# theoad/ot-vae-lightning

Hardware: AMD Instinct MI355X
Metric: training images/sec (whole node) + OT-loss rel-err vs CPU ref (higher is better)
Workload: dtype f32; 1 GPU; MNIST-32 CNN VAE (capacity 8, latent 128x1x1, residual=add) + GaussianPrior(loss_coeff=0.1): fwd+bwd+Adam + latent Gaussian statistics update, hipGraph replay; per_gpu_batch=1024, global_batch=1024, parallelism=single GPU

## Files before the change

### ot_vae_lightning_amd/csrc/conv.hip

```cpp
#include "common.h"
#include "conv_small.h"
#include "conv_tile.h"
#include "conv_wtile.h"

static inline Geom to_geom(const otvae_conv_geom* g) {
    Geom r = {g->N, g->Hs, g->Ws, g->Cs, g->up, g->Ho, g->Wo, g->Cn, g->KH, g->KW, g->stride, g->pad};
    return r;
}

static int check_geom(const otvae_conv_geom* g, const char* who) {
    OTVAE_REQUIRE(g != nullptr, "%s: geom is NULL", who);
    OTVAE_REQUIRE(g->N > 0 && g->Hs > 0 && g->Ws > 0 && g->Cs > 0 && g->Cn > 0, "%s: non-positive dims", who);
    OTVAE_REQUIRE(g->up == 1 || g->up == 2, "%s: up must be 1 or 2 (got %d)", who, g->up);
    OTVAE_REQUIRE(g->stride == 1 || g->stride == 2, "%s: stride must be 1 or 2 (got %d)", who, g->stride);
    OTVAE_REQUIRE(!(g->up == 2 && g->stride != 1), "%s: up-sampling with stride != 1 unsupported", who);
    OTVAE_REQUIRE(g->KH >= 1 && g->KH <= 7 && g->KW >= 1 && g->KW <= 7, "%s: kernel size out of range", who);
    int Hu = g->Hs * g->up, Wu = g->Ws * g->up;
    int ho = (Hu + 2 * g->pad - g->KH) / g->stride + 1, wo = (Wu + 2 * g->pad - g->KW) / g->stride + 1;
    OTVAE_REQUIRE(ho == g->Ho && wo == g->Wo, "%s: output size mismatch: geom says %dx%d, conv gives %dx%d", who,
                  g->Ho, g->Wo, ho, wo);
    OTVAE_REQUIRE((int64_t)g->N * Hu * Wu * imax(g->Cs, g->Cn) < (int64_t)1 << 31, "%s: tensor too large for 32-bit indexing",
                  who);
    OTVAE_REQUIRE(g->Cs <= 2048 && g->Cn <= 2048, "%s: more than 2048 channels unsupported", who);
    if (g->stride == 2) OTVAE_REQUIRE(g->Hs % 2 == 0 && g->Ws % 2 == 0, "%s: stride 2 needs even input size", who);
// ... 42 lines not shown
        n = rdiv(t, g.Hs, rd.iHs, rd.small);
        const int sy = t - (unsigned)n * g.Hs;
        iy = 2 * sy + (child >> 1);
        ix = 2 * sx + (child & 1);
    } else if (g.stride == 2) {
        const int W2 = g.Ws >> 1, H2 = g.Hs >> 1;
        const unsigned t = rdiv(row, W2, rd.iW2, rd.small);
        const int jx = row - t * W2;
        n = rdiv(t, H2, rd.iH2, rd.small);
        const int jy = t - (unsigned)n * H2;
        iy = 2 * jy + py;
        ix = 2 * jx + px;
    } else {
        const unsigned t = rdiv(row, g.Ws, rd.iWs, rd.small);
        ix = row - t * g.Ws;
        n = rdiv(t, g.Hs, rd.iHs, rd.small);
        iy = t - (unsigned)n * g.Hs;
    }
}

template <int NT>
struct GemmSmem {
    static constexpr int BN = 16 * NT;
    static constexpr int LDA = KC + 2;
    static constexpr int LDB = BN + ((BN % 32 == 0) ? 16 : 0);
    static constexpr size_t as_off = 0;
    static constexpr size_t bs_off = as_off + sizeof(float) * 2 * TM * LDA;
    static constexpr size_t red_off = bs_off + sizeof(float) * 2 * KC * LDB;
    static constexpr size_t tap_off = red_off + sizeof(double) * 4 * 2 * BN;
    static constexpr size_t row_off = tap_off + sizeof(int) * (3 * MAX_TAPS + 1);
    static constexpr size_t bytes = (row_off + sizeof(int) * 3 * TM + 15) / 16 * 16;
};

template <int MODE, int NT, bool VEC, bool UT = false>
__device__ __forceinline__ void conv_gemm_body(char* __restrict__ smem, const Geom& g, const float* __restrict__ S,
                                               const float* __restrict__ scale, const float* __restrict__ shift, int relu,
                                               const float* __restrict__ Bmat,
                                               const float* __restrict__ bias, const float* __restrict__ res,
                                               float* __restrict__ y,
                                               const float* __restrict__ xin, const float* __restrict__ mean,
                                               const float* __restrict__ invstd, float* __restrict__ gv,
                                               double* __restrict__ partial, int CsPad, int bx, int by, int bz, int gx,
                                               int gz) {
    using SM = GemmSmem<NT>;
    constexpr int BN = SM::BN;
    constexpr int LDA = SM::LDA;
    constexpr int LDB = SM::LDB;
    constexpr int NB_ELEMS = KC * BN / 256;
    float(*As)[TM * LDA] = reinterpret_cast<float(*)[TM * LDA]>(smem + SM::as_off);
    float(*Bs)[KC * LDB] = reinterpret_cast<float(*)[KC * LDB]>(smem + SM::bs_off);
    double* red = reinterpret_cast<double*>(smem + SM::red_off);
    int* tap_dy = reinterpret_cast<int*>(smem + SM::tap_off);
    int* tap_dx = tap_dy + MAX_TAPS;
    int* tap_w = tap_dx + MAX_TAPS;
    int& s_ntaps = tap_w[MAX_TAPS];
    int* row_n = reinterpret_cast<int*>(smem + SM::row_off);
    int* row_y = row_n + TM;
    int* row_x = row_y + TM;

    const int tid = threadIdx.x, lane = tid & 63, wave = tid >> 6;
    const int r16 = lane & 15, kq = lane >> 4;
    const int cls = bz, py = cls >> 1, px = cls & 1;
    const int Hu = g.Hs * g.up, Wu = g.Ws * g.up;
    const int CK = MODE == 0 ? g.Cs : g.Cn;
    const int NC = MODE == 0 ? g.Cn : g.Cs;
    const int n0 = by * BN;
    const int lim_y = MODE == 0 ? Hu : g.Ho * g.stride, lim_x = MODE == 0 ? Wu : g.Wo * g.stride;
    const int sh = MODE == 0 ? g.up - 1 : g.stride - 1;
    const int srcH = MODE == 0 ? g.Hs : g.Ho, srcW = MODE == 0 ? g.Ws : g.Wo;
    const unsigned rows = MODE == 0 ? (unsigned)g.N * g.Ho * g.Wo
                                    : (g.stride == 2 ? (unsigned)g.N * (g.Hs >> 1) * (g.Ws >> 1) : (unsigned)g.N * Hu * Wu);
    const unsigned ntiles = (rows + TM - 1) / TM;
    const RowDiv rd = make_rowdiv(g, rows);

    if (tid == 0) {
        int nt = 0;
        for (int kh = 0; kh < g.KH; ++kh)
            for (int kw = 0; kw < g.KW; ++kw) {
                bool ok;
                int dy, dx;
                if (MODE == 0) {
                    dy = kh - g.pad;
                    dx = kw - g.pad;
                    ok = (dy + (g.Ho - 1) * g.stride >= 0) && (dy < Hu) && (dx + (g.Wo - 1) * g.stride >= 0) && (dx < Wu);
                } else {
                    dy = g.pad - kh;
                    dx = g.pad - kw;
                    ok = true;
                    if (g.stride == 2) ok = (((py + dy) & 1) == 0) && (((px + dx) & 1) == 0);
                    ok = ok && (Hu - 1 + dy >= 0) && (dy < lim_y) && (Wu - 1 + dx >= 0) && (dx < lim_x);
                }
                if (ok) {
                    tap_dy[nt] = dy;
                    tap_dx[nt] = dx;
                    tap_w[nt] = kh * g.KW + kw;
                    ++nt;
                }
            }
        s_ntaps = nt;
    }
    __syncthreads();
    const int ntaps = s_ntaps;
    const int K = ntaps * CK;
    const int nch = (K + KC - 1) / KC;
    const float inv_ck = 1.0f / (float)CK;
    const int cpt = CK / KC;
    const float inv_cpt = 1.0f / (float)(cpt > 0 ? cpt : 1);

    const int a_kl = tid & 31, a_r0 = tid >> 5;

    double s1[NT], s2[NT];
#pragma unroll
    for (int j = 0; j < NT; ++j) s1[j] = s2[j] = 0.0;

    for (unsigned tile = bx; tile < ntiles; tile += gx) {
        __syncthreads();
        if (tid < TM) {
            const unsigned row = tile * TM + tid;
            int n = -1, ry = 0, rx = 0;
            if (row < rows) {
                if (MODE == 0) {
                    const unsigned t = rdiv(row, g.Wo, rd.iWo, rd.small);
                    const int ox = row - t * g.Wo;
                    n = rdiv(t, g.Ho, rd.iHo, rd.small);
                    const int oy = t - (unsigned)n * g.Ho;
                    ry = oy * g.stride;
                    rx = ox * g.stride;
                } else {
                    int iy, ix;
                    dgrad_row_to_pos(g, rd, row, py, px, n, iy, ix);
                    ry = iy;
                    rx = ix;
                }
            }
            row_n[tid] = n;
            row_y[tid] = ry;
            row_x[tid] = rx;
        }
        __syncthreads();

        f32x4 acc[NT];
#pragma unroll
        for (int j = 0; j < NT; ++j) acc[j] = (f32x4){0.f, 0.f, 0.f, 0.f};

        constexpr int NBV = (8 * BN + 255) / 256;
        float areg[8], breg[NB_ELEMS];
        float4 areg4[2], breg4[NBV];
        float4 a_sc4 = make_float4(1.f, 1.f, 1.f, 1.f), a_sh4 = make_float4(0.f, 0.f, 0.f, 0.f);
        int a_ok = 0;
        float a_sc = 1.f, a_sh = 0.f;
        const int v_k4 = tid & 7, v_r0 = tid >> 3;
        int vr_n[2], vr_y[2], vr_x[2];
        if constexpr (VEC) {
// ... 247 lines not shown
                const int buf = ch & 1;
                if (ch + 1 < nch) stage_load(ch + 1);
                {
                    const float* Ab = &As[buf][(wave * 16 + r16) * LDA + kq];
                    const float* Bb = &Bs[buf][kq * LDB + r16];
                    float av[KC / 4], bv[KC / 4][NT];
#pragma unroll
                    for (int ks = 0; ks < KC / 4; ++ks) {
                        av[ks] = Ab[ks * 4];
#pragma unroll
                        for (int j = 0; j < NT; ++j) bv[ks][j] = Bb[ks * 4 * LDB + j * 16];
                    }
#pragma unroll
                    for (int ks = 0; ks < KC / 4; ++ks)
#pragma unroll
                        for (int j = 0; j < NT; ++j) acc[j] = mfma16(av[ks], bv[ks][j], acc[j]);
                }
                if (ch + 1 < nch) stage_store(buf ^ 1);
                __syncthreads();
            }
        }

        const unsigned row0 = tile * TM + wave * 16 + kq * 4;
        if (MODE == 0) {
#pragma unroll
            for (int j = 0; j < NT; ++j) {
                const int col = n0 + j * 16 + r16;
                if (col < g.Cn) {
                    const float bv = bias ? bias[col] : 0.f;
#pragma unroll
                    for (int r = 0; r < 4; ++r) {
                        const unsigned pm = row0 + r;
                        if (pm < rows) {
                            const size_t o = (size_t)pm * g.Cn + col;
                            float v = acc[j][r] + bv;
                            if (res) v += res[o];
                            y[o] = v;
                            if (partial) {
                                s1[j] += (double)v;
                                s2[j] += (double)v * (double)v;
                            }
                        }
                    }
                }
            }
        } else {
#pragma unroll
            for (int j = 0; j < NT; ++j) {
                const int col = n0 + j * 16 + r16;
                if (col >= g.Cs) continue;
                const float sc = scale ? scale[col] : 1.f, shf = scale ? shift[col] : 0.f;
                const float mu = mean ? mean[col] : 0.f, is = mean ? invstd[col] : 0.f;
                if (g.up == 2) {
                    if (row0 < rows) {
                        const unsigned parent = row0 >> 2;
                        float val = (acc[j][0] + acc[j][1]) + (acc[j][2] + acc[j][3]);
                        const size_t o = (size_t)parent * g.Cs + col;
                        float xv = 0.f;
                        if (relu || mean) xv = xin[o];
                        if (relu) {
                            const float v = scale ? fmaf(xv, sc, shf) : xv;
                            val = v > 0.f ? val : 0.f;
                        }
                        gv[o] = val;
                        if (mean) {
                            s1[j] += (double)val;
                            s2[j] += (double)val * (double)((xv - mu) * is);
                        }
                    }
                } else {
#pragma unroll
                    for (int r = 0; r < 4; ++r) {
                        const unsigned rr = row0 + r;
                        if (rr < rows) {
                            size_t o;
                            if (g.stride == 1) {
                                o = (size_t)rr * g.Cs + col;
                            } else {
                                int pn, piy, pix;
                                dgrad_row_to_pos(g, rd, rr, py, px, pn, piy, pix);
                                o = ((size_t)((unsigned)pn * g.Hs + piy) * g.Ws + pix) * g.Cs + col;
                            }
                            float val = acc[j][r];
                            float xv = 0.f;
                            if (relu || mean) xv = xin[o];
                            if (relu) {
                                const float v = scale ? fmaf(xv, sc, shf) : xv;
                                val = v > 0.f ? val : 0.f;
                            }
                            gv[o] = val;
                            if (mean) {
                                s1[j] += (double)val;
                                s2[j] += (double)val * (double)((xv - mu) * is);
                            }
                        }
                    }
                }
            }
        }
    }

    if ((MODE == 1 && mean) || (MODE == 0 && partial)) {
        __syncthreads();
#pragma unroll
        for (int j = 0; j < NT; ++j) {
            double a = s1[j], b = s2[j];
            a += __shfl_xor(a, 16, 64);
            a += __shfl_xor(a, 32, 64);
            b += __shfl_xor(b, 16, 64);
            b += __shfl_xor(b, 32, 64);
            if (kq == 0) {
                red[(wave * 2 + 0) * BN + j * 16 + r16] = a;
                red[(wave * 2 + 1) * BN + j * 16 + r16] = b;
            }
        }
        __syncthreads();
        if (tid < 2 * BN) {
            const int which = tid / BN, cc = tid % BN;
            const double t = (red[(0 * 2 + which) * BN + cc] + red[(1 * 2 + which) * BN + cc]) +
                             (red[(2 * 2 + which) * BN + cc] + red[(3 * 2 + which) * BN + cc]);
            const unsigned p = bz * gx + bx;
            const unsigned Ptot = gx * gz;
            bn_stat_out(partial, which, CsPad, n0 + cc, Ptot, p, t);
        }
    }
}

template <int MODE, int NT, bool VEC, bool UT, bool TAB = false>
__global__ __launch_bounds__(256) void conv_gemm_kernel(Geom g, const float* __restrict__ S, const float* __restrict__ scale,
                                                        const float* __restrict__ shift, int relu,
                                                        const float* __restrict__ Bmat, const float* __restrict__ bias,
                                                        const float* __restrict__ res, float* __restrict__ y,
                                                        const float* __restrict__ xin, const float* __restrict__ mean,
                                                        const float* __restrict__ invstd, float* __restrict__ gv,
                                                        double* __restrict__ partial, int CsPad, BnFold fold) {
    __shared__ __align__(16) char smem[GemmSmem<NT>::bytes];
    if constexpr (TAB) {
        __shared__ __align__(16) float bn_tab[2][BN_TAB];
        bn_tab_fill(fold, scale, shift, g.Cs, bn_tab[0], bn_tab[1], (blockIdx.x | blockIdx.y | blockIdx.z) == 0);
        conv_gemm_body<MODE, NT, VEC, UT>(smem, g, S, bn_tab[0], bn_tab[1], relu, Bmat, bias, res, y, xin, mean, invstd, gv, partial, CsPad,
                                      blockIdx.x, blockIdx.y, blockIdx.z, gridDim.x, gridDim.z);
    } else {
        conv_gemm_body<MODE, NT, VEC, UT>(smem, g, S, scale, shift, relu, Bmat, bias, res, y, xin, mean, invstd, gv, partial, CsPad,
                                      blockIdx.x, blockIdx.y, blockIdx.z, gridDim.x, gridDim.z);
    }
}

template <int MODE, bool VEC, bool UT>
static void launch_gemm_v(int NT, dim3 grid, hipStream_t st, Geom g, const float* S, const float* scale, const float* shift,
                          int relu, const float* Bmat, const float* bias, const float* res, float* y, const float* xin,
                          const float* mean, const float* invstd, float* gv, double* partial, int CsPad, const BnFold& fold) {
    const bool tab = MODE == 0 && (scale != nullptr || fold.slots != nullptr) && g.Cs <= BN_TAB;
#define OTVAE_CG(N_)                                                                                                        \
    do {                                                                                                                    \
        if constexpr (MODE == 0) {                                                                                          \
            if (tab) {                                                                                                      \
                conv_gemm_kernel<MODE, N_, VEC, UT, true><<<grid, 256, 0, st>>>(g, S, scale, shift, relu, Bmat, bias, res, y, xin, mean, \
                                                                            invstd, gv, partial, CsPad, fold);              \
                break;                                                                                                      \
            }                                                                                                               \
        }                                                                                                                   \
        conv_gemm_kernel<MODE, N_, VEC, UT, false><<<grid, 256, 0, st>>>(g, S, scale, shift, relu, Bmat, bias, res, y, xin, mean, invstd, \
                                                                     gv, partial, CsPad, fold);                             \
    } while (0)
    switch (NT) {
        case 1: OTVAE_CG(1); break;
        case 2: OTVAE_CG(2); break;
        case 3: OTVAE_CG(3); break;
        default: OTVAE_CG(4); break;
    }
#undef OTVAE_CG
}

static inline bool aligned16(const void* p) { return ((uintptr_t)p & 15) == 0; }

template <int MODE>
static void launch_gemm(int NT, dim3 grid, hipStream_t st, Geom g, const float* S, const float* scale, const float* shift,
                        int relu, const float* Bmat, const float* bias, const float* res, float* y, const float* xin,
                        const float* mean, const float* invstd, float* gv, double* partial, int CsPad, const BnFold& fold = BnFold{}) {
    const bool vec = (g.Cs % 4 == 0) && (g.Cn % 4 == 0) && aligned16(S) && aligned16(Bmat) &&
                     (scale == nullptr || (aligned16(scale) && aligned16(shift)));
    const int CK = MODE == 0 ? g.Cs : g.Cn;
    if (vec && CK % KC == 0)
        launch_gemm_v<MODE, true, true>(NT, grid, st, g, S, scale, shift, relu, Bmat, bias, res, y, xin, mean, invstd, gv, partial, CsPad, fold);
    else if (vec)
        launch_gemm_v<MODE, true, false>(NT, grid, st, g, S, scale, shift, relu, Bmat, bias, res, y, xin, mean, invstd, gv, partial, CsPad, fold);
    else
        launch_gemm_v<MODE, false, false>(NT, grid, st, g, S, scale, shift, relu, Bmat, bias, res, y, xin, mean, invstd, gv, partial, CsPad, fold);
}

static void fwd_grid(const Geom& g, int& NT, dim3& grid, int& CnPad) {
    const unsigned M = (unsigned)g.N * g.Ho * g.Wo;
    NT = pick_nt(g.Cn, cdiv(M, TM));
    const int ny = cdiv(cdiv(g.Cn, 16), NT);
    grid = dim3(imin(cdiv(M, TM), 2048), ny, 1);
    CnPad = ny * 16 * NT;
}

extern "C" int otvae_conv_fwd_stats_ws(const otvae_conv_geom* gg, int* P, int* CnPad) {
    int rc = check_geom(gg, "otvae_conv_fwd_stats_ws");
    if (rc) return rc;
    Geom g = to_geom(gg);
    int NT, cp;
    dim3 grid;
    fwd_grid(g, NT, grid, cp);
    if (conv_small_ok(g)) grid.x = imin(grid.x, 1024);
    TilePlan pl;
    dim3 tg;
    size_t sm;
    if (!conv_small_ok(g) && conv_tile_plan(g, 0, pl, tg, sm)) {
        grid.x = tg.x * tg.z;
        cp = pl.cpad;
    }
    if (P) *P = grid.x;
    if (CnPad) *CnPad = cp;
    return OTVAE_OK;
}

static inline bool g_cs_le_tab(const otvae_conv_geom* g) { return g->Cs <= BN_TAB; }

static int conv_fwd_ex(const otvae_conv_geom* gg, const float* x, const float* scale, const float* shift, int relu, const float* wT,
                       const float* bias, const float* residual, float* y, double* stat_dst, const BnFold& fold, void* stream) {
    int rc = check_geom(gg, "otvae_conv_fwd");
    if (rc) return rc;
    OTVAE_REQUIRE(x && wT && y, "otvae_conv_fwd: NULL tensor");
    OTVAE_REQUIRE((scale == nullptr) == (shift == nullptr), "otvae_conv_fwd: scale and shift must be given together");
    OTVAE_REQUIRE(fold.slots == nullptr || g_cs_le_tab(gg), "otvae_conv_fwd: a folded BatchNorm takes at most %d channels", BN_TAB);
    Geom g = to_geom(gg);
    int NT, CnPad;
    dim3 grid;
    fwd_grid(g, NT, grid, CnPad);
    if (conv_small_ok(g)) {
        conv_small_fwd(g, imin(grid.x, 1024), x, scale, shift, relu, wT, bias, residual, y, stat_dst, CnPad, fold,
                       (hipStream_t)stream);
        OTVAE_CHECK_LAUNCH("otvae_conv_fwd(small)");
        return OTVAE_OK;
    }
    {
        TilePlan pl;
        dim3 tg;
        size_t sm;
        if (conv_tile_plan(g, 0, pl, tg, sm)) {
            OTVAE_REQUIRE(aligned16(x) && aligned16(wT) && aligned16(y) && (!bias || aligned16(bias)) &&
                              (!residual || aligned16(residual)) && (!scale || (aligned16(scale) && aligned16(shift))),
                          "otvae_conv_fwd: tensors of a layer with channel counts %% 4 == 0 must be 16-byte aligned");
            rc = conv_tile_fwd(pl, tg, sm, (hipStream_t)stream, x, scale, shift, relu, wT, bias, residual, y, stat_dst, fold);
            OTVAE_REQUIRE(rc == 0, "otvae_conv_fwd: no image-tile kernel for nt=%d rbw=%d", pl.nt, pl.rbw);
            OTVAE_CHECK_LAUNCH("otvae_conv_fwd(tile)");
            return OTVAE_OK;
        }
    }
    launch_gemm<0>(NT, grid, (hipStream_t)stream, g, x, scale, shift, relu, wT, bias, residual, y, nullptr, nullptr, nullptr,
                   nullptr, stat_dst, CnPad, fold);
    OTVAE_CHECK_LAUNCH("otvae_conv_fwd");
    return OTVAE_OK;
}

extern "C" int otvae_conv_fwd(const otvae_conv_geom* gg, const float* x, const float* scale, const float* shift, int relu,
                              const float* wT, const float* bias, const float* residual, float* y, double* stat_partial,
                              void* stream) {
    return conv_fwd_ex(gg, x, scale, shift, relu, wT, bias, residual, y, stat_partial, BnFold{}, stream);
}

__global__ void weight_transpose_kernel(const float* __restrict__ wT, float* __restrict__ wD, int T, int Cs, int Cn) {
    const size_t total = (size_t)T * Cs * Cn;
    for (size_t i = blockIdx.x * (size_t)blockDim.x + threadIdx.x; i < total; i += (size_t)gridDim.x * blockDim.x) {
        const int c = i % Cs;
        const size_t r = i / Cs;
        const int n = r % Cn;
        const int t = r / Cn;
        wD[i] = wT[((size_t)t * Cs + c) * Cn + n];
    }
}

extern "C" int otvae_weight_transpose(const float* wT, float* wD, int T, int Cs, int Cn, void* stream) {
    OTVAE_REQUIRE(wT && wD && T > 0 && Cs > 0 && Cn > 0, "otvae_weight_transpose: bad argument");
    const size_t total = (size_t)T * Cs * Cn;
    weight_transpose_kernel<<<imin(cdiv(total, 256), 2048), 256, 0, (hipStream_t)stream>>>(wT, wD, T, Cs, Cn);
    OTVAE_CHECK_LAUNCH("otvae_weight_transpose");
    return OTVAE_OK;
}

__global__ void weight_transpose_batched_kernel(const float* __restrict__ src_base, float* __restrict__ dst_base,
                                                const int64_t* __restrict__ table) {
    const int64_t* d = table + (size_t)blockIdx.y * 5;
    const float* wT = src_base + d[0];
    float* wD = dst_base + d[1];
    const int T = (int)d[2], Cs = (int)d[3], Cn = (int)d[4];
    const size_t total = (size_t)T * Cs * Cn;
    for (size_t i = blockIdx.x * (size_t)blockDim.x + threadIdx.x; i < total; i += (size_t)gridDim.x * blockDim.x) {
        const int c = i % Cs;
        const size_t r = i / Cs;
        const int n = r % Cn;
        const int t = r / Cn;
        wD[i] = wT[((size_t)t * Cs + c) * Cn + n];
    }
}

extern "C" int otvae_weight_transpose_batched(const float* src_base, float* dst_base, const int64_t* table, int n_layers,
                                              int64_t max_elems, void* stream) {
    OTVAE_REQUIRE(src_base && dst_base && table && n_layers > 0 && max_elems > 0, "otvae_weight_transpose_batched: bad argument");
    dim3 grid(imin(cdiv(max_elems, 256), 256), n_layers);
    weight_transpose_batched_kernel<<<grid, 256, 0, (hipStream_t)stream>>>(src_base, dst_base, table);
    OTVAE_CHECK_LAUNCH("otvae_weight_transpose_batched");
    return OTVAE_OK;
}

static void dgrad_grid(const Geom& g, int& NT, dim3& grid, int& CsPad) {
    const int Hu = g.Hs * g.up, Wu = g.Ws * g.up;
    const unsigned rows = (g.stride == 2) ? (unsigned)g.N * (g.Hs >> 1) * (g.Ws >> 1) : (unsigned)g.N * Hu * Wu;
    const int nz = g.stride == 2 ? 4 : 1;
    NT = pick_nt(g.Cs, (long)cdiv(rows, TM) * nz);
    const int ny = cdiv(cdiv(g.Cs, 16), NT);
    grid = dim3(imax(1, imin(cdiv(rows, TM), 1024 / nz)), ny, nz);
    CsPad = ny * 16 * NT;
}

extern "C" int otvae_conv_bwd_data_ws(const otvae_conv_geom* gg, int* P, int* CsPad) {
    int rc = check_geom(gg, "otvae_conv_bwd_data_ws");
    if (rc) return rc;
    Geom g = to_geom(gg);
    int NT;
    dim3 grid;
    int cp;
    dgrad_grid(g, NT, grid, cp);
    TilePlan pl;
    dim3 tg;
    size_t sm;
    if (!conv_small_ok(g) && conv_tile_plan(g, 1, pl, tg, sm)) {
        grid = tg;
        cp = pl.cpad;
    }
    if (P) *P = grid.x * grid.z;
    if (CsPad) *CsPad = cp;
    return OTVAE_OK;
}

static int conv_bwd_data_ex(const otvae_conv_geom* gg, const float* gy, const float* wD, const float* x, const float* scale,
                            const float* shift, int relu, const float* mean, const float* invstd, float* gv, double* bn_partial,
                            void* stream);

extern "C" int otvae_conv_bwd_data(const otvae_conv_geom* gg, const float* gy, const float* wD, const float* x,
                                   const float* scale, const float* shift, int relu, const float* mean, const float* invstd,
                                   float* gv, double* bn_partial, void* stream) {
    return conv_bwd_data_ex(gg, gy, wD, x, scale, shift, relu, mean, invstd, gv, bn_partial, stream);
}

static int conv_bwd_data_ex(const otvae_conv_geom* gg, const float* gy, const float* wD, const float* x, const float* scale,
                            const float* shift, int relu, const float* mean, const float* invstd, float* gv, double* bn_partial,
                            void* stream) {
    int rc = check_geom(gg, "otvae_conv_bwd_data");
    if (rc) return rc;
    OTVAE_REQUIRE(gy && wD && gv, "otvae_conv_bwd_data: NULL tensor");
    OTVAE_REQUIRE((scale == nullptr) == (shift == nullptr), "otvae_conv_bwd_data: scale/shift must come together");
    OTVAE_REQUIRE((mean == nullptr) == (invstd == nullptr), "otvae_conv_bwd_data: mean/invstd must come together");
    OTVAE_REQUIRE(!(relu || mean) || x, "otvae_conv_bwd_data: x needed for the ReLU mask / BatchNorm sums");
    OTVAE_REQUIRE(!mean || bn_partial, "otvae_conv_bwd_data: bn_partial workspace missing");
    Geom g = to_geom(gg);
    int NT, CsPad;
    dim3 grid;
    dgrad_grid(g, NT, grid, CsPad);
    if (conv_small_ok(g)) {
        conv_small_dgrad(g, grid.x * grid.z, gy, wD, x, scale, shift, relu, mean, invstd, gv, bn_partial, CsPad,
                         (hipStream_t)stream);
        OTVAE_CHECK_LAUNCH("otvae_conv_bwd_data(small)");
        return OTVAE_OK;
    }
    {
        TilePlan pl;
        dim3 tg;
        size_t sm;
        if (conv_tile_plan(g, 1, pl, tg, sm)) {
            OTVAE_REQUIRE(aligned16(gy) && aligned16(wD) && aligned16(gv) && (!x || aligned16(x)) &&
                              (!scale || (aligned16(scale) && aligned16(shift))) && (!mean || (aligned16(mean) && aligned16(invstd))),
                          "otvae_conv_bwd_data: tensors of a layer with channel counts %% 4 == 0 must be 16-byte aligned");
            rc = conv_tile_dgrad(pl, tg, sm, (hipStream_t)stream, gy, wD, x, scale, shift, relu, mean, invstd, gv, bn_partial);
            OTVAE_REQUIRE(rc == 0, "otvae_conv_bwd_data: no image-tile kernel for nt=%d rbw=%d", pl.nt, pl.rbw);
            OTVAE_CHECK_LAUNCH("otvae_conv_bwd_data(tile)");
            return OTVAE_OK;
        }
    }
    launch_gemm<1>(NT, grid, (hipStream_t)stream, g, gy, scale, shift, relu, wD, nullptr, nullptr, nullptr, x, mean, invstd, gv,
                   bn_partial, CsPad);
    OTVAE_CHECK_LAUNCH("otvae_conv_bwd_data");
    return OTVAE_OK;
}

#define PC 32
template <int NT>
struct WgradSmem {
    static constexpr int BN = 16 * NT;
    static constexpr int LDA = 64 + 16;
    static constexpr int LDB = BN + ((BN % 32 == 0) ? 16 : 0);
    static constexpr size_t at_off = 0;
    static constexpr size_t gt_off = at_off + sizeof(float) * 2 * PC * LDA;
    static constexpr size_t live_off = gt_off + sizeof(float) * 2 * PC * LDB;
    static constexpr size_t bytes = live_off + 16;
};

template <int NT, bool VEC>
__device__ __forceinline__ void conv_wgrad_body(char* __restrict__ smem, const Geom& g, const float* __restrict__ x,
                                                const float* __restrict__ scale, const float* __restrict__ shift, int relu,
                                                const float* __restrict__ gy, float* __restrict__ partial, int Kp,
                                                int has_bias, int skip_dead, unsigned chunk, int bx, int by, int bz) {
    using SM = WgradSmem<NT>;
    constexpr int BN = SM::BN;
    constexpr int LDA = SM::LDA;
    constexpr int LDB = SM::LDB;
    constexpr int NB_ELEMS = PC * BN / 256;
    float(*At)[PC * LDA] = reinterpret_cast<float(*)[PC * LDA]>(smem + SM::at_off);
    float(*Gt)[PC * LDB] = reinterpret_cast<float(*)[PC * LDB]>(smem + SM::gt_off);
    int* s_live = reinterpret_cast<int*>(smem + SM::live_off);

    const int tid = threadIdx.x, lane = tid & 63, wave = tid >> 6;
    const int r16 = lane & 15, kq = lane >> 4;
    const int kb = bx, n0 = by * BN;
// ... 530 lines not shown
            if (dead && dead[j]) {
                OTVAE_REQUIRE(Cs[j] > 0 && K[j] % Cs[j] == 0 && K[j] / Cs[j] <= 32, "otvae_wgrad_reduce_batched: entry %d: Cs", j);
                d.Cs[i] = Cs[j];
                d.dead[i] = dead[j];
            }
            const size_t total = (size_t)Kp[j] * Cn[j];
            const size_t work = P[j] < 16 ? cdiv(total, 256) : (total >= 4096 ? cdiv(total, 64) : cdiv(total, 4));
            if (work > maxwork) maxwork = work;
        }
        dim3 grid(imin((int)maxwork, 512), m);
        wgrad_reduce_batched_kernel<<<grid, 256, 0, st>>>(d);
        OTVAE_CHECK_LAUNCH("otvae_wgrad_reduce_batched");
    }
    return OTVAE_OK;
}

#define CJ_MAX 4
struct DevJob {
    Geom g;
    const float* a0;
    const float* scale;
    const float* shift;
    const float* b0;
    const float* bias;
    const float* res;
    const float* xin;
    const float* mean;
    const float* invstd;
    float* out;
    double* partial;
    int kind, NT, relu, cpad, Kp, has_bias, skip_dead;
    unsigned chunk;
    int gx, gy, gz, block0;
    BnFold fold;
};
struct DevJobs {
    int n;
    DevJob j[CJ_MAX];
};

template <bool UT>
__global__ __launch_bounds__(256) void conv_jobs_kernel(DevJobs t) {
    extern __shared__ __align__(16) char jobs_smem[];
    int ji = 0;
#pragma unroll
    for (int i = 1; i < CJ_MAX; ++i)
        if (i < t.n && (int)blockIdx.x >= t.j[i].block0) ji = i;
    const DevJob& J = t.j[ji];
    const int lb = (int)blockIdx.x - J.block0;
    const int bx = lb % J.gx;
    const int r = lb / J.gx;
    const int by = r % J.gy, bz = r / J.gy;
    __shared__ __align__(16) float bn_tab[2][BN_TAB];
    const bool fwd_norm = J.kind == OTVAE_JOB_FWD && (J.scale != nullptr || J.fold.slots != nullptr);
    if (fwd_norm) bn_tab_fill(J.fold, J.scale, J.shift, J.g.Cs, bn_tab[0], bn_tab[1], lb == 0);
    const float* const fsc = fwd_norm ? bn_tab[0] : nullptr;
    const float* const fsh = fwd_norm ? bn_tab[1] : nullptr;
#define CJ_FWD(N_)                                                                                                        \
    conv_gemm_body<0, N_, true, UT>(jobs_smem, J.g, J.a0, fsc, fsh, J.relu, J.b0, J.bias, J.res, J.out, nullptr, nullptr, \
                                nullptr, nullptr, J.partial, J.cpad, bx, by, bz, J.gx, J.gz)
#define CJ_DGRAD(N_)                                                                                                      \
    conv_gemm_body<1, N_, true, UT>(jobs_smem, J.g, J.a0, J.scale, J.shift, J.relu, J.b0, nullptr, nullptr, nullptr, J.xin,     \
                                J.mean, J.invstd, J.out, J.partial, J.cpad, bx, by, bz, J.gx, J.gz)
#define CJ_WGRAD(N_) \
    conv_wgrad_body<N_, true>(jobs_smem, J.g, J.a0, J.scale, J.shift, J.relu, J.b0, J.out, J.Kp, J.has_bias, J.skip_dead, \
                              J.chunk, bx, by, bz)
    switch (J.kind * 4 + J.NT - 1) {
        case 0: CJ_FWD(1); break;
        case 1: CJ_FWD(2); break;
        case 2: CJ_FWD(3); break;
        case 3: CJ_FWD(4); break;
        case 4: CJ_DGRAD(1); break;
        case 5: CJ_DGRAD(2); break;
        case 6: CJ_DGRAD(3); break;
        case 7: CJ_DGRAD(4); break;
        case 8: CJ_WGRAD(1); break;
        case 9: CJ_WGRAD(2); break;
        case 10: CJ_WGRAD(3); break;
        default: CJ_WGRAD(4); break;
    }
#undef CJ_FWD
#undef CJ_DGRAD
#undef CJ_WGRAD
}

static size_t job_smem_bytes(int kind, int NT) {
    if (kind == OTVAE_JOB_BWD_WEIGHT) {
        switch (NT) {
            case 1: return WgradSmem<1>::bytes;
            case 2: return WgradSmem<2>::bytes;
            case 3: return WgradSmem<3>::bytes;
            default: return WgradSmem<4>::bytes;
        }
    }
    switch (NT) {
        case 1: return GemmSmem<1>::bytes;
// ... 63 lines not shown
            const DevJob& d = pack.j[i];
            const size_t total = (size_t)d.Kp * d.g.Cn;
            wgrad_reduce_kernel<<<imin(cdiv(total, d.gz >= 32 ? 4 : 64), 2048), 256, 0, st>>>(
                jb.wpartial, d.gz, d.Kp - (jb.has_bias ? 1 : 0), d.Kp, d.g.Cn, jb.gw, jb.gb);
            OTVAE_CHECK_LAUNCH("otvae_conv_multi(reduce)");
        }
        pack = {};
        smem = 0;
        nblocks = 0;
        pack_ut = -1;
        return OTVAE_OK;
    };
    for (int i = 0; i < n; ++i) {
        const otvae_conv_job& jb = jobs[i];
        OTVAE_REQUIRE(jb.kind >= OTVAE_JOB_FWD && jb.kind <= OTVAE_JOB_BWD_WEIGHT, "otvae_conv_multi: job %d: bad kind %d", i,
                      jb.kind);
        int rc = check_geom(&jb.geom, "otvae_conv_multi");
        if (rc) return rc;
        OTVAE_REQUIRE((jb.scale == nullptr) == (jb.shift == nullptr), "otvae_conv_multi: job %d: scale/shift must come together", i);
        OTVAE_REQUIRE(jb.kind == OTVAE_JOB_FWD || (jb.fold.slots == nullptr && jb.stat_slots == nullptr),
                      "otvae_conv_multi: job %d: fold / stat_slots belong to forward jobs", i);
        Geom g = to_geom(&jb.geom);
        DevJob d = {};
        d.g = g;
        d.kind = jb.kind;
        d.relu = jb.relu;
        d.scale = jb.scale;
        d.shift = jb.shift;
        bool packable = false;
        const bool ch4 = (g.Cs % 4 == 0) && (g.Cn % 4 == 0);
        if (jb.kind == OTVAE_JOB_FWD) {
            OTVAE_REQUIRE(jb.x && jb.w && jb.y, "otvae_conv_multi: job %d (forward): NULL tensor", i);
            dim3 grid;
            fwd_grid(g, d.NT, grid, d.cpad);
            rc = bn_fold_from_abi("otvae_conv_multi", jb.fold, g.Cs, &d.fold);
            if (rc) return rc;
            OTVAE_REQUIRE(!(jb.stat_partial && jb.stat_slots), "otvae_conv_multi: job %d: statistics go to partials OR to slots", i);
            OTVAE_REQUIRE_SLOTS("otvae_conv_multi (stat_slots)", jb.stat_slots, jb.stat_nslots);
            OTVAE_REQUIRE(jb.fold.slots == nullptr || g.Cs <= BN_TAB, "otvae_conv_multi: job %d: a folded BatchNorm takes at most %d channels", i, BN_TAB);
            packable = !conv_small_ok(g) && ch4 && aligned16(jb.x) && aligned16(jb.w) &&
                       (jb.scale == nullptr || (aligned16(jb.scale) && aligned16(jb.shift))) &&
                       ((jb.scale == nullptr && jb.fold.slots == nullptr) || g.Cs <= BN_TAB);
            {
                TilePlan pl;
                dim3 tg;
                size_t sm;
                if (packable && conv_tile_plan(g, 0, pl, tg, sm)) packable = false;
            }
            d.a0 = jb.x;
            d.b0 = jb.w;
            d.bias = jb.bias;
            d.res = jb.residual;
            d.out = jb.y;
            d.partial = jb.stat_slots ? bn_tag_slots(jb.stat_slots, jb.stat_nslots) : jb.stat_partial;
            d.gx = grid.x, d.gy = grid.y, d.gz = grid.z;
        } else if (jb.kind == OTVAE_JOB_BWD_DATA) {
            OTVAE_REQUIRE(jb.gy && jb.w && jb.gv, "otvae_conv_multi: job %d (data gradient): NULL tensor", i);
            OTVAE_REQUIRE((jb.mean == nullptr) == (jb.invstd == nullptr), "otvae_conv_multi: job %d: mean/invstd must come together", i);
            OTVAE_REQUIRE(!(jb.relu || jb.mean) || jb.x, "otvae_conv_multi: job %d: x needed for the ReLU mask / BatchNorm sums", i);
            OTVAE_REQUIRE(!jb.mean || jb.bn_partial || jb.bn_slots, "otvae_conv_multi: job %d: bn_partial workspace / bn_slots missing", i);
            OTVAE_REQUIRE(!(jb.bn_partial && jb.bn_slots), "otvae_conv_multi: job %d: BatchNorm-backward sums go to partials OR to slots", i);
            OTVAE_REQUIRE_SLOTS("otvae_conv_multi (bn_slots)", jb.bn_slots, jb.bn_nslots);
            dim3 grid;
            dgrad_grid(g, d.NT, grid, d.cpad);
            packable = !conv_small_ok(g) && ch4 && aligned16(jb.gy) && aligned16(jb.w);
            {
                TilePlan pl;
                dim3 tg;
                size_t sm;
                if (packable && conv_tile_plan(g, 1, pl, tg, sm)) packable = false;
            }
            d.a0 = jb.gy;
            d.b0 = jb.w;
            d.xin = jb.x;
            d.mean = jb.mean;
            d.invstd = jb.invstd;
            d.out = jb.gv;
            d.partial = jb.bn_slots ? bn_tag_slots(jb.bn_slots, jb.bn_nslots) : jb.bn_partial;
            d.gx = grid.x, d.gy = grid.y, d.gz = grid.z;
        } else {
            OTVAE_REQUIRE(jb.x && jb.gy && jb.wpartial && jb.gw, "otvae_conv_multi: job %d (weight gradient): NULL tensor", i);
            OTVAE_REQUIRE(!jb.has_bias || jb.gb, "otvae_conv_multi: job %d: gb missing", i);
            int P, nkb, nnb;
            wgrad_plan(g, jb.has_bias, d.NT, P, d.chunk, nkb, nnb, d.Kp);
            packable = !conv_small_wgrad_ok(g) && ch4 && aligned16(jb.x) && aligned16(jb.gy) &&
                       (jb.scale == nullptr || (aligned16(jb.scale) && aligned16(jb.shift)));
            {
                WTilePlan wp;
                int nbk;
                size_t sm;
                if (conv_wtile_plan(g, jb.has_bias, wp, nbk, sm)) packable = false;
            }
            d.a0 = jb.x;
            d.b0 = jb.gy;
            d.out = jb.wpartial;
            d.has_bias = jb.has_bias;
            d.skip_dead = jb.defer_reduce == OTVAE_DEFER_SPARSE;
// ... 24 lines not shown
```

### ot_vae_lightning_amd/functional.py

```python
from __future__ import annotations

import ctypes as C
import math
import os
from typing import List, Optional, Sequence, Tuple

import torch
from torch import Tensor

from . import _lib
from . import ops as _ops
from ._lib import ConvGeom, check, ptr, ptr_array, stream

BN_EPS = 1e-5
BN_MOMENTUM = 0.1


def is_nhwc(x: Tensor) -> bool:
    if x.dim() != 4:
        return False
    n, c, h, w = x.shape
    want = (h * w * c, 1, w * c, c)
    for size, st, ws in zip(x.shape, x.stride(), want):
        if size != 1 and st != ws:
# ... 21 lines not shown
    if is_hwio(w):
        return w
    return w.permute(2, 3, 1, 0).contiguous().permute(3, 2, 0, 1)


def new_hwio(co: int, ci: int, kh: int, kw: int, device=None, dtype=torch.float32) -> Tensor:
    return torch.empty((kh, kw, ci, co), device=device, dtype=dtype).permute(3, 2, 0, 1)


def _grad_buffer(param: Optional[Tensor], like: Tensor) -> Tensor:
    if param is not None:
        getter = getattr(param, "_otvae_grad_view", None)
        if getter is not None:
            return getter()
    return torch.empty_strided(like.shape, like.stride(), device=like.device, dtype=like.dtype)


def _geom(x: Tensor, weight: Tensor, stride: int, pad: int, up: int) -> Tuple[ConvGeom, int, int]:
    n, cs, hs, ws = x.shape
    cn, ci, kh, kw = weight.shape
    if ci != cs:
        raise ValueError(f"conv: input has {cs} channels but weight expects {ci}")
    ho = (hs * up + 2 * pad - kh) // stride + 1
    wo = (ws * up + 2 * pad - kw) // stride + 1
    return ConvGeom(n, hs, ws, cs, up, ho, wo, cn, kh, kw, stride, pad), ho, wo


_PLAN_CACHE: dict = {}


def _conv_plan(g: ConvGeom, has_bias: bool):
    env = os.environ
    key = (g.N, g.Hs, g.Ws, g.Cs, g.up, g.Ho, g.Wo, g.Cn, g.KH, g.KW, g.stride, g.pad, has_bias,
           "OTVAE_NO_TILE" in env, "OTVAE_NO_WTILE" in env, "OTVAE_TILE_ALL" in env, "OTVAE_WTILE_ALL" in env)
    plan = _PLAN_CACHE.get(key)
    if plan is None:
        lib = _lib.load()
        p_s, ld, p_w, p_d, cp, dead = C.c_int(0), C.c_int(0), C.c_int(0), C.c_int(0), C.c_int(0), C.c_uint32(0)
        check(lib.otvae_conv_fwd_stats_ws(C.byref(g), C.byref(p_s), C.byref(ld)), "otvae_conv_fwd_stats_ws")
        check(lib.otvae_conv_bwd_weight_ws(C.byref(g), int(has_bias), C.byref(p_w)), "otvae_conv_bwd_weight_ws")
        check(lib.otvae_conv_bwd_data_ws(C.byref(g), C.byref(p_d), C.byref(cp)), "otvae_conv_bwd_data_ws")
        check(lib.otvae_conv_dead_taps(C.byref(g), C.byref(dead)), "otvae_conv_dead_taps")
        plan = _PLAN_CACHE[key] = (p_s.value, ld.value, p_w.value, p_d.value, cp.value, dead.value)
    return plan


class BNBranch:
    __slots__ = ("gamma", "beta", "running_mean", "running_var", "num_batches_tracked")

    def __init__(self, gamma, beta, running_mean=None, running_var=None, num_batches_tracked=None):
        self.gamma, self.beta = gamma, beta
        self.running_mean, self.running_var, self.num_batches_tracked = running_mean, running_var, num_batches_tracked


BN_SLOTS_MODE = int(os.environ.get("OTVAE_BN_SLOTS", "1"))


class Slots:
    __slots__ = ("buf", "ld", "n")

    def __init__(self, buf: Tensor, ld: int, n: int):
        self.buf, self.ld, self.n = buf, int(ld), int(n)


class SlotArena:
    _state: dict = {}
    WORDS = 1 << 20
# ... 1704 lines not shown
```

Measured before the change: 396,600 images/s.

## Split small-spatial conv GEMMs into per-position classes to skip padding taps

For implicit-GEMM convs whose output (forward) or input (data-grad) spatial size is at most 16 positions, each output position gets its own grid z-class. Each class's tap list then holds only the kernel taps that fall inside the image, so the K loop skips work that was multiplying zero padding. A heuristic counts live taps with and without classes and enables the split only when it reduces them, and an env var can turn it off. The jobs kernel also copies the selected job struct by value instead of indexing with a runtime variable. The trade-off is more blocks with fewer rows each (rows = N) and output writes strided by the class count.

```diff
diff --git a/ot_vae_lightning_amd/csrc/conv.hip b/ot_vae_lightning_amd/csrc/conv.hip
--- a/ot_vae_lightning_amd/csrc/conv.hip
+++ b/ot_vae_lightning_amd/csrc/conv.hip
@@ -98,6 +98,28 @@
     static constexpr size_t bytes = (row_off + sizeof(int) * 3 * TM + 15) / 16 * 16;
 };
 
+__host__ __device__ __forceinline__ bool gemm_tap_live(const Geom& g, int mode, int pcls, int cls, int kh, int kw) {
+    const int Hu = g.Hs * g.up, Wu = g.Ws * g.up;
+    if (mode == 0) {
+        const int dy = kh - g.pad, dx = kw - g.pad;
+        if (pcls) {
+            const int ay = (cls / g.Wo) * g.stride, ax = (cls % g.Wo) * g.stride;
+            return ay + dy >= 0 && ay + dy < Hu && ax + dx >= 0 && ax + dx < Wu;
+        }
+        return (dy + (g.Ho - 1) * g.stride >= 0) && (dy < Hu) && (dx + (g.Wo - 1) * g.stride >= 0) && (dx < Wu);
+    }
+    const int dy = g.pad - kh, dx = g.pad - kw;
+    const int lim_y = g.Ho * g.stride, lim_x = g.Wo * g.stride;
+    if (pcls) {
+        const int ty = cls / g.Ws + dy, tx = cls % g.Ws + dx;
+        return ty >= 0 && ty < lim_y && tx >= 0 && tx < lim_x && (g.stride == 1 || ((ty & 1) == 0 && (tx & 1) == 0));
+    }
+    const int py = cls >> 1, px = cls & 1;
+    bool ok = true;
+    if (g.stride == 2) ok = (((py + dy) & 1) == 0) && (((px + dx) & 1) == 0);
+    return ok && (Hu - 1 + dy >= 0) && (dy < lim_y) && (Wu - 1 + dx >= 0) && (dx < lim_x);
+}
+
 template <int MODE, int NT, bool VEC, bool UT = false>
 __device__ __forceinline__ void conv_gemm_body(char* __restrict__ smem, const Geom& g, const float* __restrict__ S,
                                                const float* __restrict__ scale, const float* __restrict__ shift, int relu,
@@ -107,7 +129,7 @@
                                                const float* __restrict__ xin, const float* __restrict__ mean,
                                                const float* __restrict__ invstd, float* __restrict__ gv,
                                                double* __restrict__ partial, int CsPad, int bx, int by, int bz, int gx,
-                                               int gz) {
+                                               int gz, int pcls) {
     using SM = GemmSmem<NT>;
     constexpr int BN = SM::BN;
     constexpr int LDA = SM::LDA;
@@ -134,8 +156,11 @@
     const int lim_y = MODE == 0 ? Hu : g.Ho * g.stride, lim_x = MODE == 0 ? Wu : g.Wo * g.stride;
     const int sh = MODE == 0 ? g.up - 1 : g.stride - 1;
     const int srcH = MODE == 0 ? g.Hs : g.Ho, srcW = MODE == 0 ? g.Ws : g.Wo;
-    const unsigned rows = MODE == 0 ? (unsigned)g.N * g.Ho * g.Wo
-                                    : (g.stride == 2 ? (unsigned)g.N * (g.Hs >> 1) * (g.Ws >> 1) : (unsigned)g.N * Hu * Wu);
+    const int cW = MODE == 0 ? g.Wo : g.Ws;
+    const int cy = pcls ? cls / cW : 0, cx = pcls ? cls - (cls / cW) * cW : 0;
+    const unsigned rows = pcls ? (unsigned)g.N
+                               : MODE == 0 ? (unsigned)g.N * g.Ho * g.Wo
+                                           : (g.stride == 2 ? (unsigned)g.N * (g.Hs >> 1) * (g.Ws >> 1) : (unsigned)g.N * Hu * Wu);
     const unsigned ntiles = (rows + TM - 1) / TM;
     const RowDiv rd = make_rowdiv(g, rows);
 
@@ -143,22 +168,9 @@
         int nt = 0;
         for (int kh = 0; kh < g.KH; ++kh)
             for (int kw = 0; kw < g.KW; ++kw) {
-                bool ok;
-                int dy, dx;
-                if (MODE == 0) {
-                    dy = kh - g.pad;
-                    dx = kw - g.pad;
-                    ok = (dy + (g.Ho - 1) * g.stride >= 0) && (dy < Hu) && (dx + (g.Wo - 1) * g.stride >= 0) && (dx < Wu);
-                } else {
-                    dy = g.pad - kh;
-                    dx = g.pad - kw;
-                    ok = true;
-                    if (g.stride == 2) ok = (((py + dy) & 1) == 0) && (((px + dx) & 1) == 0);
-                    ok = ok && (Hu - 1 + dy >= 0) && (dy < lim_y) && (Wu - 1 + dx >= 0) && (dx < lim_x);
-                }
-                if (ok) {
-                    tap_dy[nt] = dy;
-                    tap_dx[nt] = dx;
+                if (gemm_tap_live(g, MODE, pcls, cls, kh, kw)) {
+                    tap_dy[nt] = MODE == 0 ? kh - g.pad : g.pad - kh;
+                    tap_dx[nt] = MODE == 0 ? kw - g.pad : g.pad - kw;
                     tap_w[nt] = kh * g.KW + kw;
                     ++nt;
                 }
@@ -184,7 +196,11 @@
         if (tid < TM) {
             const unsigned row = tile * TM + tid;
             int n = -1, ry = 0, rx = 0;
-            if (row < rows) {
+            if (row < rows && pcls) {
+                n = row;
+                ry = MODE == 0 ? cy * g.stride : cy;
+                rx = MODE == 0 ? cx * g.stride : cx;
+            } else if (row < rows) {
                 if (MODE == 0) {
                     const unsigned t = rdiv(row, g.Wo, rd.iWo, rd.small);
                     const int ox = row - t * g.Wo;
@@ -498,7 +514,7 @@
                     for (int r = 0; r < 4; ++r) {
                         const unsigned pm = row0 + r;
                         if (pm < rows) {
-                            const size_t o = (size_t)pm * g.Cn + col;
+                            const size_t o = (pcls ? (size_t)pm * pcls + cls : (size_t)pm) * g.Cn + col;
                             float v = acc[j][r] + bv;
                             if (res) v += res[o];
                             y[o] = v;
@@ -540,7 +556,9 @@
                         const unsigned rr = row0 + r;
                         if (rr < rows) {
                             size_t o;
-                            if (g.stride == 1) {
+                            if (pcls) {
+                                o = ((size_t)rr * pcls + cls) * g.Cs + col;
+                            } else if (g.stride == 1) {
                                 o = (size_t)rr * g.Cs + col;
                             } else {
                                 int pn, piy, pix;
@@ -599,35 +617,36 @@
                                                         const float* __restrict__ res, float* __restrict__ y,
                                                         const float* __restrict__ xin, const float* __restrict__ mean,
                                                         const float* __restrict__ invstd, float* __restrict__ gv,
-                                                        double* __restrict__ partial, int CsPad, BnFold fold) {
+                                                        double* __restrict__ partial, int CsPad, BnFold fold, int pcls) {
     __shared__ __align__(16) char smem[GemmSmem<NT>::bytes];
     if constexpr (TAB) {
         __shared__ __align__(16) float bn_tab[2][BN_TAB];
         bn_tab_fill(fold, scale, shift, g.Cs, bn_tab[0], bn_tab[1], (blockIdx.x | blockIdx.y | blockIdx.z) == 0);
         conv_gemm_body<MODE, NT, VEC, UT>(smem, g, S, bn_tab[0], bn_tab[1], relu, Bmat, bias, res, y, xin, mean, invstd, gv, partial, CsPad,
-                                      blockIdx.x, blockIdx.y, blockIdx.z, gridDim.x, gridDim.z);
+                                      blockIdx.x, blockIdx.y, blockIdx.z, gridDim.x, gridDim.z, pcls);
     } else {
         conv_gemm_body<MODE, NT, VEC, UT>(smem, g, S, scale, shift, relu, Bmat, bias, res, y, xin, mean, invstd, gv, partial, CsPad,
-                                      blockIdx.x, blockIdx.y, blockIdx.z, gridDim.x, gridDim.z);
+                                      blockIdx.x, blockIdx.y, blockIdx.z, gridDim.x, gridDim.z, pcls);
     }
 }
 
 template <int MODE, bool VEC, bool UT>
 static void launch_gemm_v(int NT, dim3 grid, hipStream_t st, Geom g, const float* S, const float* scale, const float* shift,
                           int relu, const float* Bmat, const float* bias, const float* res, float* y, const float* xin,
-                          const float* mean, const float* invstd, float* gv, double* partial, int CsPad, const BnFold& fold) {
+                          const float* mean, const float* invstd, float* gv, double* partial, int CsPad, const BnFold& fold,
+                          int pcls) {
     const bool tab = MODE == 0 && (scale != nullptr || fold.slots != nullptr) && g.Cs <= BN_TAB;
 #define OTVAE_CG(N_)                                                                                                        \
     do {                                                                                                                    \
         if constexpr (MODE == 0) {                                                                                          \
             if (tab) {                                                                                                      \
                 conv_gemm_kernel<MODE, N_, VEC, UT, true><<<grid, 256, 0, st>>>(g, S, scale, shift, relu, Bmat, bias, res, y, xin, mean, \
-                                                                            invstd, gv, partial, CsPad, fold);              \
+                                                                            invstd, gv, partial, CsPad, fold, pcls);        \
                 break;                                                                                                      \
             }                                                                                                               \
         }                                                                                                                   \
         conv_gemm_kernel<MODE, N_, VEC, UT, false><<<grid, 256, 0, st>>>(g, S, scale, shift, relu, Bmat, bias, res, y, xin, mean, invstd, \
-                                                                     gv, partial, CsPad, fold);                             \
+                                                                     gv, partial, CsPad, fold, pcls);                       \
     } while (0)
     switch (NT) {
         case 1: OTVAE_CG(1); break;
@@ -643,19 +662,48 @@
 template <int MODE>
 static void launch_gemm(int NT, dim3 grid, hipStream_t st, Geom g, const float* S, const float* scale, const float* shift,
                         int relu, const float* Bmat, const float* bias, const float* res, float* y, const float* xin,
-                        const float* mean, const float* invstd, float* gv, double* partial, int CsPad, const BnFold& fold = BnFold{}) {
+                        const float* mean, const float* invstd, float* gv, double* partial, int CsPad, int pcls,
+                        const BnFold& fold = BnFold{}) {
     const bool vec = (g.Cs % 4 == 0) && (g.Cn % 4 == 0) && aligned16(S) && aligned16(Bmat) &&
                      (scale == nullptr || (aligned16(scale) && aligned16(shift)));
     const int CK = MODE == 0 ? g.Cs : g.Cn;
     if (vec && CK % KC == 0)
-        launch_gemm_v<MODE, true, true>(NT, grid, st, g, S, scale, shift, relu, Bmat, bias, res, y, xin, mean, invstd, gv, partial, CsPad, fold);
+        launch_gemm_v<MODE, true, true>(NT, grid, st, g, S, scale, shift, relu, Bmat, bias, res, y, xin, mean, invstd, gv, partial, CsPad, fold, pcls);
     else if (vec)
-        launch_gemm_v<MODE, true, false>(NT, grid, st, g, S, scale, shift, relu, Bmat, bias, res, y, xin, mean, invstd, gv, partial, CsPad, fold);
+        launch_gemm_v<MODE, true, false>(NT, grid, st, g, S, scale, shift, relu, Bmat, bias, res, y, xin, mean, invstd, gv, partial, CsPad, fold, pcls);
     else
-        launch_gemm_v<MODE, false, false>(NT, grid, st, g, S, scale, shift, relu, Bmat, bias, res, y, xin, mean, invstd, gv, partial, CsPad, fold);
-}
-
-static void fwd_grid(const Geom& g, int& NT, dim3& grid, int& CnPad) {
+        launch_gemm_v<MODE, false, false>(NT, grid, st, g, S, scale, shift, relu, Bmat, bias, res, y, xin, mean, invstd, gv, partial, CsPad, fold, pcls);
+}
+
+static int gemm_classes(const Geom& g, int mode) {
+    if (conv_small_ok(g)) return 0;
+    const char* e = getenv("OTVAE_CONV_CLASSES");
+    if (e && e[0] == '0' && e[1] == 0) return 0;
+    if (mode == 1 && g.up != 1) return 0;
+    const int P = mode == 0 ? g.Ho * g.Wo : g.Hs * g.Ws;
+    if (P > 16) return 0;
+    long before = 0, after = 0;
+    for (int c = 0; c < P; ++c) {
+        const int par = (mode == 1 && g.stride == 2) ? ((c / g.Ws) & 1) * 2 + ((c % g.Ws) & 1) : 0;
+        for (int kh = 0; kh < g.KH; ++kh)
+            for (int kw = 0; kw < g.KW; ++kw) {
+                before += gemm_tap_live(g, mode, 0, par, kh, kw);
+                after += gemm_tap_live(g, mode, P, c, kh, kw);
+            }
+    }
+    return after < before ? P : 0;
+}
+
+static void fwd_grid(const Geom& g, int& NT, dim3& grid, int& CnPad, int& pcls) {
+    pcls = gemm_classes(g, 0);
+    if (pcls) {
+        const int tiles = cdiv(g.N, TM);
+        NT = pick_nt(g.Cn, (long)tiles * pcls);
+        const int ny = cdiv(cdiv(g.Cn, 16), NT);
+        grid = dim3(imax(1, imin(tiles, 2048 / pcls)), ny, pcls);
+        CnPad = ny * 16 * NT;
+        return;
+    }
     const unsigned M = (unsigned)g.N * g.Ho * g.Wo;
     NT = pick_nt(g.Cn, cdiv(M, TM));
     const int ny = cdiv(cdiv(g.Cn, 16), NT);
@@ -667,18 +715,19 @@
     int rc = check_geom(gg, "otvae_conv_fwd_stats_ws");
     if (rc) return rc;
     Geom g = to_geom(gg);
-    int NT, cp;
+    int NT, cp, pcls;
     dim3 grid;
-    fwd_grid(g, NT, grid, cp);
+    fwd_grid(g, NT, grid, cp, pcls);
     if (conv_small_ok(g)) grid.x = imin(grid.x, 1024);
     TilePlan pl;
     dim3 tg;
     size_t sm;
     if (!conv_small_ok(g) && conv_tile_plan(g, 0, pl, tg, sm)) {
         grid.x = tg.x * tg.z;
+        grid.z = 1;
         cp = pl.cpad;
     }
-    if (P) *P = grid.x;
+    if (P) *P = grid.x * grid.z;
     if (CnPad) *CnPad = cp;
     return OTVAE_OK;
 }
@@ -693,9 +742,9 @@
     OTVAE_REQUIRE((scale == nullptr) == (shift == nullptr), "otvae_conv_fwd: scale and shift must be given together");
     OTVAE_REQUIRE(fold.slots == nullptr || g_cs_le_tab(gg), "otvae_conv_fwd: a folded BatchNorm takes at most %d channels", BN_TAB);
     Geom g = to_geom(gg);
-    int NT, CnPad;
+    int NT, CnPad, pcls;
     dim3 grid;
-    fwd_grid(g, NT, grid, CnPad);
+    fwd_grid(g, NT, grid, CnPad, pcls);
     if (conv_small_ok(g)) {
         conv_small_fwd(g, imin(grid.x, 1024), x, scale, shift, relu, wT, bias, residual, y, stat_dst, CnPad, fold,
                        (hipStream_t)stream);
@@ -717,7 +766,7 @@
         }
     }
     launch_gemm<0>(NT, grid, (hipStream_t)stream, g, x, scale, shift, relu, wT, bias, residual, y, nullptr, nullptr, nullptr,
-                   nullptr, stat_dst, CnPad, fold);
+                   nullptr, stat_dst, CnPad, pcls, fold);
     OTVAE_CHECK_LAUNCH("otvae_conv_fwd");
     return OTVAE_OK;
 }
@@ -772,7 +821,16 @@
     return OTVAE_OK;
 }
 
-static void dgrad_grid(const Geom& g, int& NT, dim3& grid, int& CsPad) {
+static void dgrad_grid(const Geom& g, int& NT, dim3& grid, int& CsPad, int& pcls) {
+    pcls = gemm_classes(g, 1);
+    if (pcls) {
+        const int tiles = cdiv(g.N, TM);
+        NT = pick_nt(g.Cs, (long)tiles * pcls);
+        const int ny = cdiv(cdiv(g.Cs, 16), NT);
+        grid = dim3(imax(1, imin(tiles, 1024 / pcls)), ny, pcls);
+        CsPad = ny * 16 * NT;
+        return;
+    }
     const int Hu = g.Hs * g.up, Wu = g.Ws * g.up;
     const unsigned rows = (g.stride == 2) ? (unsigned)g.N * (g.Hs >> 1) * (g.Ws >> 1) : (unsigned)g.N * Hu * Wu;
     const int nz = g.stride == 2 ? 4 : 1;
@@ -786,10 +844,10 @@
     int rc = check_geom(gg, "otvae_conv_bwd_data_ws");
     if (rc) return rc;
     Geom g = to_geom(gg);
-    int NT;
+    int NT, pcls;
     dim3 grid;
     int cp;
-    dgrad_grid(g, NT, grid, cp);
+    dgrad_grid(g, NT, grid, cp, pcls);
     TilePlan pl;
     dim3 tg;
     size_t sm;
@@ -823,9 +881,9 @@
     OTVAE_REQUIRE(!(relu || mean) || x, "otvae_conv_bwd_data: x needed for the ReLU mask / BatchNorm sums");
     OTVAE_REQUIRE(!mean || bn_partial, "otvae_conv_bwd_data: bn_partial workspace missing");
     Geom g = to_geom(gg);
-    int NT, CsPad;
+    int NT, CsPad, pcls;
     dim3 grid;
-    dgrad_grid(g, NT, grid, CsPad);
+    dgrad_grid(g, NT, grid, CsPad, pcls);
     if (conv_small_ok(g)) {
         conv_small_dgrad(g, grid.x * grid.z, gy, wD, x, scale, shift, relu, mean, invstd, gv, bn_partial, CsPad,
                          (hipStream_t)stream);
@@ -847,7 +905,7 @@
         }
     }
     launch_gemm<1>(NT, grid, (hipStream_t)stream, g, gy, scale, shift, relu, wD, nullptr, nullptr, nullptr, x, mean, invstd, gv,
-                   bn_partial, CsPad);
+                   bn_partial, CsPad, pcls);
     OTVAE_CHECK_LAUNCH("otvae_conv_bwd_data");
     return OTVAE_OK;
 }
@@ -1444,6 +1502,7 @@
     int kind, NT, relu, cpad, Kp, has_bias, skip_dead;
     unsigned chunk;
     int gx, gy, gz, block0;
+    int pcls;
     BnFold fold;
 };
 struct DevJobs {
@@ -1454,11 +1513,10 @@
 template <bool UT>
 __global__ __launch_bounds__(256) void conv_jobs_kernel(DevJobs t) {
     extern __shared__ __align__(16) char jobs_smem[];
-    int ji = 0;
+    DevJob J = t.j[0];
 #pragma unroll
     for (int i = 1; i < CJ_MAX; ++i)
-        if (i < t.n && (int)blockIdx.x >= t.j[i].block0) ji = i;
-    const DevJob& J = t.j[ji];
+        if (i < t.n && (int)blockIdx.x >= t.j[i].block0) J = t.j[i];
     const int lb = (int)blockIdx.x - J.block0;
     const int bx = lb % J.gx;
     const int r = lb / J.gx;
@@ -1470,10 +1528,10 @@
     const float* const fsh = fwd_norm ? bn_tab[1] : nullptr;
 #define CJ_FWD(N_)                                                                                                        \
     conv_gemm_body<0, N_, true, UT>(jobs_smem, J.g, J.a0, fsc, fsh, J.relu, J.b0, J.bias, J.res, J.out, nullptr, nullptr, \
-                                nullptr, nullptr, J.partial, J.cpad, bx, by, bz, J.gx, J.gz)
+                                nullptr, nullptr, J.partial, J.cpad, bx, by, bz, J.gx, J.gz, J.pcls)
 #define CJ_DGRAD(N_)                                                                                                      \
     conv_gemm_body<1, N_, true, UT>(jobs_smem, J.g, J.a0, J.scale, J.shift, J.relu, J.b0, nullptr, nullptr, nullptr, J.xin,     \
-                                J.mean, J.invstd, J.out, J.partial, J.cpad, bx, by, bz, J.gx, J.gz)
+                                J.mean, J.invstd, J.out, J.partial, J.cpad, bx, by, bz, J.gx, J.gz, J.pcls)
 #define CJ_WGRAD(N_) \
     conv_wgrad_body<N_, true>(jobs_smem, J.g, J.a0, J.scale, J.shift, J.relu, J.b0, J.out, J.Kp, J.has_bias, J.skip_dead, \
                               J.chunk, bx, by, bz)
@@ -1603,7 +1661,7 @@
         if (jb.kind == OTVAE_JOB_FWD) {
             OTVAE_REQUIRE(jb.x && jb.w && jb.y, "otvae_conv_multi: job %d (forward): NULL tensor", i);
             dim3 grid;
-            fwd_grid(g, d.NT, grid, d.cpad);
+            fwd_grid(g, d.NT, grid, d.cpad, d.pcls);
             rc = bn_fold_from_abi("otvae_conv_multi", jb.fold, g.Cs, &d.fold);
             if (rc) return rc;
             OTVAE_REQUIRE(!(jb.stat_partial && jb.stat_slots), "otvae_conv_multi: job %d: statistics go to partials OR to slots", i);
@@ -1633,7 +1691,7 @@
             OTVAE_REQUIRE(!(jb.bn_partial && jb.bn_slots), "otvae_conv_multi: job %d: BatchNorm-backward sums go to partials OR to slots", i);
             OTVAE_REQUIRE_SLOTS("otvae_conv_multi (bn_slots)", jb.bn_slots, jb.bn_nslots);
             dim3 grid;
-            dgrad_grid(g, d.NT, grid, d.cpad);
+            dgrad_grid(g, d.NT, grid, d.cpad, d.pcls);
             packable = !conv_small_ok(g) && ch4 && aligned16(jb.gy) && aligned16(jb.w);
             {
                 TilePlan pl;
diff --git a/ot_vae_lightning_amd/functional.py b/ot_vae_lightning_amd/functional.py
--- a/ot_vae_lightning_amd/functional.py
+++ b/ot_vae_lightning_amd/functional.py
@@ -77,7 +77,8 @@
 def _conv_plan(g: ConvGeom, has_bias: bool):
     env = os.environ
     key = (g.N, g.Hs, g.Ws, g.Cs, g.up, g.Ho, g.Wo, g.Cn, g.KH, g.KW, g.stride, g.pad, has_bias,
-           "OTVAE_NO_TILE" in env, "OTVAE_NO_WTILE" in env, "OTVAE_TILE_ALL" in env, "OTVAE_WTILE_ALL" in env)
+           "OTVAE_NO_TILE" in env, "OTVAE_NO_WTILE" in env, "OTVAE_TILE_ALL" in env, "OTVAE_WTILE_ALL" in env,
+           env.get("OTVAE_CONV_CLASSES"))
     plan = _PLAN_CACHE.get(key)
     if plan is None:
         lib = _lib.load()
```

Result: faster. 401,100 images/s, median of 6 (+1.1%).
